# OpenVVC/OpenVVC

Hardware: AMD Instinct MI355X
Metric: decoded frames/sec, full rcn back-end decode step (H2D of the recorded picture + MC incl. BDOF/DMVR/affine-PROF/GPM/CIIP + LMCS + inverse transform + ordered intra pass + deblocking + SAO + ALF/CC-ALF + D2H of refined MVs + wait + per-picture digest + publication to the device DPB), 4K 10-bit RA rec (higher is better)
Workload: dtype u16 samples / int16 coefficients / int32 accumulate

## Files before the change

### include/ovvc_hip.h

```cpp
#ifndef OVVC_HIP_H
#define OVVC_HIP_H

#include <stddef.h>
#include <stdint.h>

#ifdef __cplusplus
extern "C" {
#endif

#define OVHIP_ABI_VERSION 8

#define OVHIP_OK        0
#define OVHIP_ENODEV   (-1)
#define OVHIP_ENOMEM   (-2)
#define OVHIP_EINVAL   (-3)
#define OVHIP_ELAUNCH  (-4)
#define OVHIP_EUNSUP   (-5)
#define OVHIP_EREF     (-6)

enum { OVHIP_DST_VII = 0, OVHIP_DCT_VIII = 1, OVHIP_DCT_II = 2 };

typedef struct ovhip_pic {
    uint16_t *y, *cb, *cr;
    int32_t   w, h;
// ... 358 lines not shown
int   ovhip_rec_cu_inter(ovhip_recorder *rec, const ovhip_pu_desc *pu, const ovhip_affine_desc *aff);
int   ovhip_rec_ciip(ovhip_recorder *rec, int32_t x0, int32_t y0, int32_t log2_w, int32_t log2_h,
                     int32_t mode_abv, int32_t mode_lft);
int   ovhip_ciip_weight(int32_t mode_abv, int32_t mode_lft);
int   ovhip_rec_lmcs_region(ovhip_recorder *rec, int32_t x0, int32_t y0, uint32_t abv_mask, uint32_t lft_mask);
typedef struct ovhip_dbf_edge {
    uint16_t ux, uy;
    uint16_t word;
    uint8_t  comp;
    uint8_t  pad;
} ovhip_dbf_edge;
#define OVHIP_DBF_MAX_OFFSETS 8
typedef struct ovhip_dbf_offsets { int8_t beta[OVHIP_DBF_MAX_OFFSETS], tc[OVHIP_DBF_MAX_OFFSETS]; } ovhip_dbf_offsets;
const ovhip_dbf_edge *ovhip_rec_dbf_edges(const ovhip_recorder *rec, int dir, size_t *n, ovhip_dbf_offsets *offsets);
int64_t ovhip_dbf_compact(const ovhip_dbf_planes *planes, int dir, ovhip_dbf_edge *out, size_t cap);

int   ovhip_rec_dbf_ctu(ovhip_recorder *rec, const ovhip_dbf_ctu *ctu);
typedef struct ovhip_dbf_view {
    const uint64_t *ctb_bound_ver, *ctb_bound_hor, *ctb_bound_ver_c, *ctb_bound_hor_c, *aff_edg_ver, *aff_edg_hor;
    const uint64_t *bs2_ver, *bs2_hor, *bs2c_ver, *bs2c_hor, *bs1_ver, *bs1_hor, *bs1cb_ver, *bs1cb_hor, *bs1cr_ver, *bs1cr_hor, *affine_ver, *affine_hor;
    const uint8_t  *qp_y, *qp_cb, *qp_cr;
    int16_t  beta_offset, tc_offset;
    uint8_t  disable_v, disable_h, log2_ctu_s, last_x, last_y, ctu_lft, ctu_abv, pad;
    uint16_t ctu_w, ctu_h, ctb_x, ctb_y;
} ovhip_dbf_view;
int   ovhip_rec_dbf_row(ovhip_recorder *rec, const ovhip_dbf_view *ctus, size_t n);
int   ovhip_rec_dbf_mv_prepass_view(const ovhip_dbf_view *ctu, uint64_t *bs1_ver, uint64_t *bs1_hor, const ovhip_dbf_mv_ctx *mv);
int   ovhip_rec_dbf_planes(const ovhip_recorder *rec, ovhip_dbf_planes *out);
enum { OVHIP_REC_TB = 0, OVHIP_REC_COEF, OVHIP_REC_MC, OVHIP_REC_MCX, OVHIP_REC_AFF, OVHIP_REC_SIDE, OVHIP_REC_REGION,
       OVHIP_REC_CIIP, OVHIP_REC_EDGE_V, OVHIP_REC_EDGE_H, OVHIP_REC_ITASK };
// ... 368 lines not shown
```

### openvvc_amd/capi.py

```python
from __future__ import annotations

import ctypes as C
import os
from pathlib import Path

import numpy as np

_PKG = Path(__file__).resolve().parent
LIB_PATH = _PKG / os.environ.get("OVVC_HIP_LIB_NAME", "libovvc_hip.so")

OVHIP_ABI_VERSION = 8
OVHIP_OK, OVHIP_ENODEV, OVHIP_ENOMEM, OVHIP_EINVAL, OVHIP_ELAUNCH, OVHIP_EUNSUP, OVHIP_EREF = 0, -1, -2, -3, -4, -5, -6
DST_VII, DCT_VIII, DCT_II = 0, 1, 2
TB_TR, TB_DC, TB_TS, TB_TS_RAW = 0, 1, 2, 3
TB_FLAG_RASTER = 0x80
RES_ADD, RES_SUB, RES_ADD_HALF, RES_SUB_HALF, RES_SCALE = 0, 1, 2, 3, 4
MC_HPEL_FILT, MC_FILT_4x4, MC_NO_LUMA, MC_NO_CHROMA, MC_LMCS, MC_BDOF, MC_DMVR = 1, 2, 4, 8, 16, 32, 64
PU_BDOF, PU_DMVR, PU_GPM = 1, 2, 4
MC_GPM = 128


class Pic(C.Structure):
    _fields_ = [("y", C.c_void_p), ("cb", C.c_void_p), ("cr", C.c_void_p),
                ("w", C.c_int32), ("h", C.c_int32), ("stride_y", C.c_int32), ("stride_c", C.c_int32)]
# ... 161 lines not shown
               [("beta_offset", C.c_int16), ("tc_offset", C.c_int16), ("disable_v", C.c_uint8), ("disable_h", C.c_uint8), ("log2_ctu_s", C.c_uint8),
                ("last_x", C.c_uint8), ("last_y", C.c_uint8), ("ctu_lft", C.c_uint8), ("ctu_abv", C.c_uint8), ("pad", C.c_uint8),
                ("ctu_w", C.c_uint16), ("ctu_h", C.c_uint16), ("ctb_x", C.c_uint16), ("ctb_y", C.c_uint16)]


FE_BEGIN, FE_REF, FE_DMVR_ROWS, FE_DMVR_BEGIN, FE_DMVR_COLLECT, FE_SUBMIT, FE_FAIL = range(1, 8)
FRAME_EVENT_DTYPE = np.dtype([("op", "<u4"), ("frame", "<i4"), ("key", "<u8"), ("tag", "<u8"), ("a", "<i8"), ("b", "<i8"), ("result", "<i8")])
assert FRAME_EVENT_DTYPE.itemsize == 48
FRAME_TRACE_FN = C.CFUNCTYPE(None, C.c_void_p, C.c_void_p)

DBF_PLANE_NAMES = ("luma_v", "luma_h", "cb_v", "cr_v", "cb_h", "cr_h")


class DbfOffsets(C.Structure):
    _fields_ = [("beta", C.c_int8 * 8), ("tc", C.c_int8 * 8)]


class BandCounts(C.Structure):
    _fields_ = [(n, C.c_uint32) for n in ("n_tb", "n_coef", "n_mc", "n_mcx", "n_aff", "n_side", "n_reg", "n_itask", "n_edge_v", "n_edge_h")]


class JobParams(C.Structure):
    _fields_ = [("lmcs", C.c_void_p), ("sao", C.c_void_p), ("alf_ctus", C.c_void_p),
                ("alf_luma_coeff", C.c_void_p), ("alf_luma_clip", C.c_void_p),
                ("alf_chroma_coeff", C.c_void_p), ("alf_chroma_clip", C.c_void_p), ("alf_cc_coeff", C.c_void_p),
                ("log2_ctu_s", C.c_int32), ("stages", C.c_uint32), ("wait_events", C.POINTER(C.c_void_p)), ("n_wait_events", C.c_uint32),
                ("before_launch", C.c_void_p), ("before_launch_user", C.c_void_p), ("tmvp_cells", C.c_uint32), ("wait_on_host", C.c_uint32),
                ("flow_workers", C.c_uint32)]


# ... 210 lines not shown
        "ovhip_d2h": (C.c_int, [vp, vp, vp, C.c_size_t]),
        "ovhip_pic_alloc": (C.c_int, [vp, i32, i32, P(Pic)]),
        "ovhip_pic_free": (C.c_int, [vp, P(Pic)]),
        "ovhip_pic_upload": (C.c_int, [vp, P(Pic), vp, vp, vp, i32, i32]),
        "ovhip_pic_download": (C.c_int, [vp, P(Pic), vp, vp, vp, i32, i32]),
        "ovhip_itx_launch": (C.c_int, [vp, P(Pic), vp, u32, vp, vp]),
        "ovhip_mc_launch": (C.c_int, [vp, P(Pic), P(Pic), u32, vp, u32, vp, P(Pic)]),
        "ovhip_ciip_weight": (C.c_int, [C.c_int32, C.c_int32]),
        "ovhip_mcx_launch": (C.c_int, [vp, P(Pic), P(Pic), u32, vp, u32, vp, vp]),
        "ovhip_mca_launch": (C.c_int, [vp, P(Pic), P(Pic), u32, vp, u32, vp, vp]),
        "ovhip_mcxa_launch": (C.c_int, [vp, P(Pic), P(Pic), u32, vp, u32, vp, vp, u32, vp, vp]),
        "ovhip_rec_create_ex": (vp, [i32, i32, vp]),
        "ovhip_rec_set_dense_dbf_planes": (None, [vp, C.c_int]),
        "ovhip_rec_dbf_edges": (vp, [vp, C.c_int, P(C.c_size_t), P(DbfOffsets)]),
        "ovhip_dbf_launch_edges_ex": (C.c_int, [vp, P(Pic), vp, u32, vp, u32, P(DbfOffsets)]),
        "ovhip_dmvr_search_launch": (C.c_int, [vp, P(Pic), P(Pic), u32, vp, u32, vp]),
        "ovhip_rec_append_raw": (C.c_int, [vp, C.c_int, vp, C.c_size_t]),
        "ovhip_itx_launch_classes_res": (C.c_int, [vp, P(Pic), P(Pic), vp, u32, u32, vp, vp]),
        "ovhip_intra_level_launch": (C.c_int, [vp, P(Pic), P(Pic), vp, u32, vp, vp, vp, i32, u32]),
        "ovhip_intra_level_geom": (u32, [vp, C.c_size_t]),
        "ovhip_intra_sync_words": (C.c_size_t, [i32, i32, i32]),
        "ovhip_intra_flow_words": (C.c_size_t, [i32, i32]),
        "ovhip_intra_flow_items": (C.c_size_t, [vp, C.c_size_t, vp, C.c_size_t]),
        "ovhip_intra_flow_launch": (C.c_int, [vp, P(Pic), P(Pic), vp, u32, vp, u32, vp, vp, vp, i32, vp, u32, vp, i32, i32]),
        "ovhip_intra_ctu_launch": (C.c_int, [vp, P(Pic), P(Pic), vp, vp, u32, vp, vp, vp, i32, vp, u32, vp]),
        "ovhip_rec_itask_levels": (u32, [vp]),
        "ovhip_rec_isp_cu": (C.c_int, [vp, vp, vp]),
        "ovhip_isp_geometry": (None, [i32, i32, i32, P(i32), P(i32), P(i32), P(i32)]),
        "ovhip_job_bind": (C.c_int, [vp, vp]),
        "ovhip_rec_set_ctu_size": (C.c_int, [vp, i32]),
# ... 116 lines not shown
        fn.restype, fn.argtypes = res, args
    if lib.ovhip_abi_version() != OVHIP_ABI_VERSION and not ab_build:
        raise RuntimeError("libovvc_hip.so ABI version mismatch")
    if path is None:
        _lib = lib
    return lib


EXPORTED_SYMBOLS = [
    "ovhip_abi_version", "ovhip_rec_create", "ovhip_rec_destroy", "ovhip_rec_reset", "ovhip_rec_tu",
    "ovhip_rec_pu", "ovhip_rec_cu_inter", "ovhip_rec_dbf_row", "ovhip_rec_dbf_mv_prepass_view", "ovhip_rec_dbf_ctu", "ovhip_rec_dbf_planes", "ovhip_dbf_launch", "ovhip_sao_launch", "ovhip_alf_launch", "ovhip_rec_tb_cmds", "ovhip_rec_coefs", "ovhip_rec_mc_units", "ovhip_rec_mcx_units", "ovhip_mcx_launch", "ovhip_rec_affine_cu", "ovhip_rec_transform_tree", "ovhip_rec_lmcs_region", "ovhip_dbf_compact", "ovhip_rec_dbf_mv_prepass", "ovhip_dbf_launch_edges", "ovhip_rec_ciip", "ovhip_ciip_weight", "ovhip_rec_ciip_units", "ovhip_ciip_launch", "ovhip_rec_lmcs_regions", "ovhip_rec_tb_cmds_split", "ovhip_itx_launch_classes", "ovhip_itx_launch_chroma_lmcs", "ovhip_lmcs_build", "ovhip_lmcs_scale_launch", "ovhip_lmcs_inverse_launch", "ovhip_rec_aff_units", "ovhip_rec_aff_side", "ovhip_mca_launch", "ovhip_mcxa_launch", "ovhip_ctx_create",
    "ovhip_ctx_destroy", "ovhip_ctx_sync", "ovhip_ctx_shares_queue", "ovhip_ctx_new_stream", "ovhip_ctx_fork", "ovhip_ctx_join", "ovhip_last_error", "ovhip_ctx_stream", "ovhip_malloc",
    "ovhip_free", "ovhip_h2d", "ovhip_d2h", "ovhip_pic_alloc", "ovhip_pic_free", "ovhip_pic_upload",
    "ovhip_pic_download", "ovhip_itx_launch", "ovhip_mc_launch",
    "ovhip_rec_create_ex", "ovhip_rec_set_dense_dbf_planes", "ovhip_rec_dbf_edges", "ovhip_dbf_launch_edges_ex",
    "ovhip_dmvr_search_launch", "ovhip_rec_append_raw", "ovhip_rec_set_dbf_offsets", "ovhip_rec_tu_intra", "ovhip_rec_itasks", "ovhip_rec_itasks_sorted", "ovhip_itx_launch_classes_res", "ovhip_intra_level_launch", "ovhip_intra_level_geom", "ovhip_intra_sync_words", "ovhip_intra_ctu_launch", "ovhip_intra_flow_words", "ovhip_intra_flow_items", "ovhip_intra_flow_launch",
    "ovhip_rec_itask_levels", "ovhip_rec_isp_cu", "ovhip_isp_geometry", "ovhip_rec_itasks_by_ctu", "ovhip_rec_set_ctu_size", "ovhip_job_bind", "ovhip_job_create", "ovhip_job_destroy", "ovhip_job_recorder", "ovhip_job_begin",
    "ovhip_frame_band", "ovhip_frame_band_upto", "ovhip_frame_dmvr_rows_begin_upto", "ovhip_job_dmvr_rows_begin_upto", "ovhip_frame_set_band_mode", "ovhip_frame_band_stats", "ovhip_dpb_post_rows", "ovhip_dpb_rows_tag",
    "ovhip_job_band", "ovhip_job_band_active", "ovhip_job_band_busy", "ovhip_job_band_reserve", "ovhip_job_reserve_for_picture", "ovhip_rec_reserve_for_picture", "ovhip_job_band_progress", "ovhip_rec_counts", "ovhip_sao_launch_rows", "ovhip_alf_launch_rows",
    "ovhip_job_flush", "ovhip_job_wait", "ovhip_job_refined_mvs", "ovhip_job_dmvr_rows", "ovhip_job_dmvr_rows_begin", "ovhip_job_dmvr_rows_collect", "ovhip_job_last_stats", "ovhip_job_time_stage", "ovhip_job_stage_time",
    "ovhip_output_bytes", "ovhip_output_rows", "ovhip_output_pack_launch", "ovhip_output_row_md5_launch", "ovhip_output_bands", "ovhip_output_tree_md5_launch", "ovhip_pic_output", "ovhip_pic_digest",
    "ovhip_md5_init", "ovhip_md5_update", "ovhip_md5_final", "ovhip_tmvp_cells_launch", "ovhip_job_tmvp_cells", "ovhip_intra_flow_untag_launch", "ovhip_lmcs_inverse_untag_launch", "ovhip_lmcs_scale_prepare_launch",
    "ovhip_host_alloc", "ovhip_host_free", "ovhip_d2d", "ovhip_job_test_abort_next_flow",
    "ovhip_dpb_create", "ovhip_dpb_create_ex", "ovhip_dpb_destroy", "ovhip_dpb_n_devices", "ovhip_dpb_device", "ovhip_dpb_begin", "ovhip_dpb_want",
    "ovhip_dpb_publish", "ovhip_dpb_acquire", "ovhip_dpb_wait_copy", "ovhip_dpb_poll_tag", "ovhip_frame_refs_ready", "ovhip_dpb_set_unknown_key_timeout", "ovhip_dpb_unpin", "ovhip_dpb_release", "ovhip_dpb_lookup", "ovhip_dpb_shutdown",
    "ovhip_dpb_get_stats", "ovhip_dpb_begin_tag", "ovhip_dpb_want_tag", "ovhip_dpb_acquire_tag", "ovhip_frame_begin_tag", "ovhip_frame_ref_tag", "ovhip_frame_set_trace",
    "ovhip_rccl_unique_id", "ovhip_rccl_create", "ovhip_rccl_destroy", "ovhip_rccl_xfer", "ovhip_rccl_last_error", "ovhip_rccl_stats", "ovhip_rccl_self_exchange",
    "ovhip_frame_create", "ovhip_frame_destroy", "ovhip_frame_ctx", "ovhip_frame_job", "ovhip_frame_recorder", "ovhip_frame_begin", "ovhip_frame_ref",
    "ovhip_frame_ref_at", "ovhip_frame_dmvr_rows", "ovhip_frame_dmvr_rows_begin", "ovhip_frame_dmvr_rows_collect", "ovhip_frame_submit", "ovhip_frame_fail", "ovhip_frame_last_error",
    "ovhip_calllog_create", "ovhip_calllog_destroy", "ovhip_calllog_reset", "ovhip_calllog_data", "ovhip_rec_set_calllog", "ovhip_calllog_replay",
# ... 217 lines not shown
```

### openvvc_amd/csrc/kernels_dbf.hip

```cpp
#include "ovvc_common.hip.h"
#define OVT_ATTR __device__
#include "vvc_dbf_tables.h"

#ifndef OV_WPE_DBF
#define OV_WPE_DBF 0
#endif
#if OV_WPE_DBF > 0
#define OV_OCC_DBF __attribute__((amdgpu_waves_per_eu(OV_WPE_DBF)))
#else
#define OV_OCC_DBF
#endif

namespace {

struct Lim { int tc, beta; };

__device__ __forceinline__ Lim dbf_limits(int qp, int bs, int tc_off, int beta_off)
{
    Lim l;
    l.tc = ovt_dbf_tc[ov_clip3(qp + 2 * (bs - 1) + tc_off, 0, 66)];
    l.beta = (int)ovt_dbf_beta[ov_clip3(qp + beta_off, 0, 64)] << 2;
    return l;
}

// ... 308 lines not shown
        const int cw = DIR ? w4 : (w4 + 1) >> 1, chh = DIR ? (h4 + 1) >> 1 : h4;
        const uint16_t *plane = DIR ? (comp == 1 ? pl.cb_h : pl.cr_h) : (comp == 1 ? pl.cb_v : pl.cr_v);
        for (int tid = blockIdx.x * 256 + threadIdx.x; tid < cw * chh; tid += nthreads) {
            const int cx = tid % cw, cy = tid / cw;
            const int v = plane[tid];
            if (!(v & OVHIP_DBF_C_ON)) continue;
            const int ux = DIR ? cx : cx * 2, uy = DIR ? cy * 2 : cy;
            if ((DIR ? uy : ux) == 0) continue;
            const Lim lim = dbf_limits(v >> 8, 1 + !!(v & OVHIP_DBF_C_BS2), pl.tc_offset, pl.beta_offset);
            uint16_t *p = (comp == 1 ? pic.cb : pic.cr) + (uy * 2) * pic.stride_c + ux * 2;
            chroma_segment(p, DIR ? pic.stride_c : 1, DIR ? 1 : pic.stride_c, lim, v & OVHIP_DBF_C_LARGE, v & OVHIP_DBF_C_CTB_B);
        }
    }
}

template <int DIR>
__global__ __launch_bounds__(256) OV_OCC_DBF void k_dbf_list(ovhip_pic pic, const ovhip_dbf_edge *__restrict__ edges, uint32_t n,
                                                  uint64_t tc_pack, uint64_t beta_pack)
{
    const uint32_t tid = ov_xcd_slot(blockIdx.x, gridDim.x) * 256 + threadIdx.x;
    const uint32_t ei = tid >> 2;
    const int l = tid & 3;
    if (ei >= n) return;
    const ovhip_dbf_edge e = edges[ei];
    const int v = e.word;
    const int osh = (e.pad & 7) * 8;
    const int tc_offset = (int8_t)(tc_pack >> osh), beta_offset = (int8_t)(beta_pack >> osh);
    if (e.comp == 0) {
        const Lim lim = dbf_limits(v >> 8, v & 3, tc_offset, beta_offset);
        if (!(lim.tc || lim.beta)) return;
        uint16_t *p = pic.y + (e.uy * 4) * pic.stride_y + e.ux * 4 + l * (DIR ? 1 : pic.stride_y);
        luma_quad<DIR>(p, DIR ? pic.stride_y : 1, lim, (v >> 2) & 7, (v >> 5) & 7);
    } else {
        const Lim lim = dbf_limits(v >> 8, 1 + !!(v & OVHIP_DBF_C_BS2), tc_offset, beta_offset);
        uint16_t *p = (e.comp == 1 ? pic.cb : pic.cr) + (e.uy * 2) * pic.stride_c + e.ux * 2 + (l & 1) * (DIR ? 1 : pic.stride_c);
        chroma_quad<DIR>(p, DIR ? pic.stride_c : 1, lim, v & OVHIP_DBF_C_LARGE, v & OVHIP_DBF_C_CTB_B, l < 2);
    }
}

}

extern "C" int ovhip_dbf_launch_edges_ex(ovhip_ctx *ctx, const ovhip_pic *pic, const ovhip_dbf_edge *d_edges_v, uint32_t n_v,
                                         const ovhip_dbf_edge *d_edges_h, uint32_t n_h, const ovhip_dbf_offsets *offsets)
{
    if (!ctx || !pic || !offsets) return OVHIP_EINVAL;
    OV_DEVICE(ctx);
    if ((n_v && !d_edges_v) || (n_h && !d_edges_h))
        return ov_fail(ctx, OVHIP_EINVAL, "ovhip_dbf_launch_edges: null edge list", hipSuccess);
    uint64_t tc_pack, beta_pack;
    memcpy(&tc_pack, offsets->tc, 8); memcpy(&beta_pack, offsets->beta, 8);
    if (n_v) {
        hipLaunchKernelGGL(k_dbf_list<0>, dim3((n_v + 63) / 64), dim3(256), 0, ctx->stream, *pic, d_edges_v, n_v, tc_pack, beta_pack);
        OV_LAUNCH_CHECK(ctx, "k_dbf_list<v>");
    }
    if (n_h) {
        hipLaunchKernelGGL(k_dbf_list<1>, dim3((n_h + 63) / 64), dim3(256), 0, ctx->stream, *pic, d_edges_h, n_h, tc_pack, beta_pack);
        OV_LAUNCH_CHECK(ctx, "k_dbf_list<h>");
    }
    return OVHIP_OK;
}

extern "C" int ovhip_dbf_launch_edges(ovhip_ctx *ctx, const ovhip_pic *pic, const ovhip_dbf_edge *d_edges_v, uint32_t n_v,
                                      const ovhip_dbf_edge *d_edges_h, uint32_t n_h, int32_t beta_offset, int32_t tc_offset)
{
    if (beta_offset < -128 || beta_offset > 127 || tc_offset < -128 || tc_offset > 127) return OVHIP_EINVAL;
    ovhip_dbf_offsets o;
    for (int i = 0; i < OVHIP_DBF_MAX_OFFSETS; ++i) { o.beta[i] = (int8_t)beta_offset; o.tc[i] = (int8_t)tc_offset; }
    return ovhip_dbf_launch_edges_ex(ctx, pic, d_edges_v, n_v, d_edges_h, n_h, &o);
}

extern "C" int ovhip_dbf_launch(ovhip_ctx *ctx, const ovhip_pic *pic, const ovhip_dbf_planes *pl)
{
    if (!ctx || !pic || !pl) return OVHIP_EINVAL;
    OV_DEVICE(ctx);
// ... 14 lines not shown
```

### openvvc_amd/csrc/ovvc_picture.hip

```cpp
#include "ovvc_common.hip.h"
#include <stdlib.h>

extern "C" int ovhip_dmvr_search_launch(ovhip_ctx *ctx, const ovhip_pic *geom, const ovhip_pic *refs, uint32_t n_refs,
                                        const ovhip_mc_unit *d_units, uint32_t n_units, int32_t *d_mv_out);

struct BandState;
namespace {

struct DevBuf { void *p; size_t cap; };

enum { B_TB, B_COEF, B_MC, B_MCX, B_MV, B_AFF, B_SIDE, B_REG, B_SCALE, B_EV, B_EH, B_PARAM, B_CLASS, B_CIIP, B_ITASK, B_ICTU, B_IITEM, B_TMVP, B_COUNT };

struct ParamLayout { size_t sao, alf_ctus, lcoef, lclip, ccoef, cclip, cc, fwd, bwd, total; };

}

struct ovhip_job {
    ovhip_ctx *ctx;
    ovhip_ctx *home;
    int32_t w, h;
    ovhip_recorder *rec;
    DevBuf dev[B_COUNT];
    ovhip_pic tmp;
    ovhip_pic res;
// ... 5 lines not shown
    int32_t *mv_host; size_t mv_cap;
    struct { int valid, has_intra; ovhip_pic dst, refs[16], intra; uint32_t n_refs; ovhip_job_params pr; } again;
    uint32_t n_retries;
    int flow_launched;
    int test_abort, test_abort_seen;
    ovhip_tmvp_cell *tmvp_host; size_t tmvp_cap, n_tmvp;
    size_t n_mv;
    size_t dmvr_first;
    size_t rows_end; int rows_pending;
    hipEvent_t ev_rows;
    hipEvent_t ev_h2d, ev_done;
    hipStream_t up;
    int flow_on_device;
    int flushed;
    const void *packed_prev[24];
    int resident;
    ovhip_job_stats st;
    struct BandState *bs;
    int t_stage;
    hipEvent_t t_ev[32][2]; uint8_t t_pending[32]; int t_next;
    double t_sum_ms; uint64_t t_count;
};

static void band_free(ovhip_job *j);
static int  band_reset(ovhip_job *j);
static int  band_active(const ovhip_job *j);
static int  band_wait_done(ovhip_job *j);

enum { FLOW_DEVS = 64, FLOW_DECAY = 512 };
static int g_flow_shift[FLOW_DEVS], g_flow_clean[FLOW_DEVS];
// ... 88 lines not shown
    return OVHIP_OK;
}

int pinned_reserve(ovhip_job *j, void **p, size_t *cap, size_t bytes)
{
    if (bytes <= *cap) return OVHIP_OK;
    size_t nc = *cap ? *cap : 4096;
    while (nc < bytes) nc *= 2;
    void *q = pinned_alloc(nullptr, nc);
    if (!q) return ov_fail(j->ctx, OVHIP_ENOMEM, "hipHostMalloc", hipSuccess);
    if (*p) { memcpy(q, *p, *cap); pinned_free(nullptr, *p); }
    *p = q; *cap = nc;
    return OVHIP_OK;
}

extern "C" const ovhip_tb_cmd *ovhip_rec_tb_cmds_split_tiny_(ovhip_recorder *r, size_t counts[4], size_t tiny[4][4], size_t *n);
extern "C" int ovhip_itx_launch_ex_(ovhip_ctx *ctx, const ovhip_pic *dst, const ovhip_pic *res, const ovhip_tb_cmd *d_cmds, uint32_t n_large,
                                    uint32_t n_small, const uint32_t tiny3[4], const int16_t *d_coefs, const int16_t *d_lmcs_scales, const uint16_t *d_bwd_lut);

#define CHK(x) do { int r__ = (x); if (r__ != OVHIP_OK) return r__; } while (0)

#ifndef OVHIP_PACK_LIMIT
#define OVHIP_PACK_LIMIT (1 << 20)
#endif

double host_now_us()
{
    timespec t;
    clock_gettime(CLOCK_MONOTONIC, &t);
    return 1e6 * (double)t.tv_sec + 1e-3 * (double)t.tv_nsec;
// ... 401 lines not shown
    const int sao_on = pr->sao && (stages & OVHIP_STAGE_SAO), alf_on = pr->alf_ctus && (stages & OVHIP_STAGE_ALF);
    if (alf_on && (!pr->alf_luma_coeff || !pr->alf_luma_clip || !pr->alf_chroma_coeff || !pr->alf_chroma_clip || !pr->alf_cc_coeff))
        return ov_fail(ctx, OVHIP_EINVAL, "ovhip_job_flush: ALF tables missing", hipSuccess);
    ParamLayout L;
    size_t o = 0;
    auto put = [&o](size_t bytes) { size_t at = o; o += (bytes + 255) & ~(size_t)255; return at; };
    L.sao = put(sao_on ? n_ctu * sizeof(ovhip_sao_ctu) : 0);
    L.alf_ctus = put(alf_on ? n_ctu * sizeof(ovhip_alf_ctu) : 0);
    L.lcoef = put(alf_on ? 24 * OVHIP_ALF_LUMA_SET_SIZE * 2 : 0);
    L.lclip = put(alf_on ? 24 * OVHIP_ALF_LUMA_SET_SIZE * 2 : 0);
    L.ccoef = put(alf_on ? 8 * 7 * 2 : 0);
    L.cclip = put(alf_on ? 8 * 7 * 2 : 0);
    L.cc = put(alf_on ? 2 * 4 * 8 * 2 : 0);
    L.fwd = put(pr->lmcs ? 2048 : 0);
    L.bwd = put(pr->lmcs ? 2048 : 0);
#ifdef OVHIP_TUNING
    static const size_t PACK_LIMIT = getenv("OVHIP_X_PACK_LIMIT") ? (size_t)atol(getenv("OVHIP_X_PACK_LIMIT")) : (size_t)OVHIP_PACK_LIMIT;
#else
    const size_t PACK_LIMIT = OVHIP_PACK_LIMIT;
#endif
    struct Small { const void *host; size_t bytes; int buf; size_t at; } small[] = {
        { mc, n_mc * sizeof(*mc), B_MC, 0 }, { tb, n_tb * sizeof(*tb), B_TB, 0 }, { coef, n_coef * sizeof(*coef), B_COEF, 0 },
        { it, n_it * sizeof(*it), B_ITASK, 0 }, { ictu, n_ictu * sizeof(*ictu), B_ICTU, 0 },
        { j->items_host, by_flow ? n_items * sizeof(uint32_t) : 0, B_IITEM, 0 },
        { mcx, n_mcx * sizeof(*mcx), B_MCX, 0 }, { ciip, n_ciip * sizeof(*ciip), B_CIIP, 0 }, { aff, n_aff * sizeof(*aff), B_AFF, 0 },
        { side, n_side * sizeof(*side), B_SIDE, 0 }, { reg, n_reg * sizeof(*reg), B_REG, 0 },
        { ev, (stages & OVHIP_STAGE_DBF) ? n_ev * sizeof(*ev) : 0, B_EV, 0 }, { eh, (stages & OVHIP_STAGE_DBF) ? n_eh * sizeof(*eh) : 0, B_EH, 0 },
    };
    static_assert(B_COUNT <= 24, "packed_prev");
    const void *packed[24] = { nullptr };
    for (auto &sm : small) if (sm.bytes && sm.bytes <= PACK_LIMIT && !j->resident) sm.at = put(sm.bytes) + 1;
    L.total = o;
    if (L.total) {
        CHK(pinned_reserve(j, (void **)&j->param_host, &j->param_cap, L.total));
        char *ph = j->param_host;
        for (auto &sm : small) if (sm.at) memcpy(ph + sm.at - 1, sm.host, sm.bytes);
        if (sao_on) memcpy(ph + L.sao, pr->sao, n_ctu * sizeof(ovhip_sao_ctu));
        if (alf_on) {
            memcpy(ph + L.alf_ctus, pr->alf_ctus, n_ctu * sizeof(ovhip_alf_ctu));
            memcpy(ph + L.lcoef, pr->alf_luma_coeff, 24 * OVHIP_ALF_LUMA_SET_SIZE * 2);
            memcpy(ph + L.lclip, pr->alf_luma_clip, 24 * OVHIP_ALF_LUMA_SET_SIZE * 2);
            memcpy(ph + L.ccoef, pr->alf_chroma_coeff, 8 * 7 * 2);
            memcpy(ph + L.cclip, pr->alf_chroma_clip, 8 * 7 * 2);
            memcpy(ph + L.cc, pr->alf_cc_coeff, 2 * 4 * 8 * 2);
        }
        if (pr->lmcs) { memcpy(ph + L.fwd, pr->lmcs->fwd_lut, 2048); memcpy(ph + L.bwd, pr->lmcs->bwd_lut, 2048); }
    }

    const double t_flush1 = host_now_us();
    j->up = (j->resident || no_upload) ? nullptr : upload_stream_for(j);
    if (j->up) {
        hipError_t e0 = hipSuccess;
        if (j->flushed) e0 = hipStreamWaitEvent(j->up, j->ev_done, 0);
        if (e0 == hipSuccess && j->rows_pending) e0 = hipStreamWaitEvent(j->up, j->ev_rows, 0);
        if (e0 != hipSuccess) { j->up = nullptr; return ov_fail(ctx, OVHIP_ENODEV, "ovhip_job_flush: upload stream", e0); }
    }
    {
    StageTimer t_(j, OVHIP_TIME_H2D);
    CHK(h2d(j, B_PARAM, j->param_host, L.total));
    if (n_mcx) {
        CHK(dev_reserve(j, B_MV, n_mcx * 16));
        CHK(pinned_reserve(j, (void **)&j->mv_host, &j->mv_cap, n_mcx * 16));
    }
    if (n_reg) CHK(dev_reserve(j, B_SCALE, n_reg * 2));
    for (auto &sm : small) {
        if (j->resident) continue;
        if (sm.at) packed[sm.buf] = (const char *)j->dev[B_PARAM].p + sm.at - 1;
        else CHK(h2d(j, sm.buf, sm.host, sm.bytes));
    }
    }
    if (no_upload) memcpy(packed, j->packed_prev, sizeof(packed)); else { memcpy(j->packed_prev, packed, sizeof(packed)); j->flow_on_device = by_flow && n_items; }
    auto DEV = [&](int k) -> const void * { return packed[k] ? packed[k] : j->dev[k].p; };
    if (j->up) {
        hipStream_t up = j->up; j->up = nullptr;
        OV_HIP(ctx, hipEventRecord(j->ev_h2d, up));
        OV_HIP(ctx, hipStreamWaitEvent(ctx->stream, j->ev_h2d, 0));
    } else OV_HIP(ctx, hipEventRecord(j->ev_h2d, ctx->stream));
    const double t_flush2 = host_now_us();
    for (uint32_t i = 0; i < pr->n_wait_events; ++i)
        if (pr->wait_events && pr->wait_events[i]) {
            if (pr->wait_on_host) OV_HIP(ctx, hipEventSynchronize((hipEvent_t)pr->wait_events[i]));
            else OV_HIP(ctx, hipStreamWaitEvent(ctx->stream, (hipEvent_t)pr->wait_events[i], 0));
        }
    if (pr->before_launch && pr->before_launch(pr->before_launch_user))
        return ov_fail(ctx, OVHIP_EINVAL, "ovhip_job_flush: before_launch callback failed", hipSuccess);
#ifdef OVHIP_TUNING
    static const int X_H2D_HOSTWAIT = getenv("OVHIP_X_H2D_HOSTWAIT") ? atoi(getenv("OVHIP_X_H2D_HOSTWAIT")) : 0;
    static const int X_MV_D2H = getenv("OVHIP_X_MV_D2H") ? atoi(getenv("OVHIP_X_MV_D2H")) : 3;
    if (X_H2D_HOSTWAIT && !j->resident) OV_HIP(ctx, hipEventSynchronize(j->ev_h2d));
#else
    const int X_MV_D2H = 3;
#endif
// ... 139 lines not shown
        }
        for (uint32_t l = 0; by_level && !by_flow && l < n_lv; ++l) {
            const uint32_t a = lv_start[l], b = lv_start[l + 1];
            if (b > a) {
                CHK(ovhip_intra_level_launch(ctx, dst, &j->res, d_it + a, b - a, (const ovhip_lmcs_region *)DEV(B_REG), pr->lmcs,
                                             (int16_t *)j->dev[B_SCALE].p, log2_ctu, ovhip_intra_level_geom(it + a, b - a)));
                j->st.n_launches++;
            }
        }
        const bool inverse = pr->lmcs && (stages & OVHIP_STAGE_ITX);
        if (inverse) { CHK(ovhip_lmcs_inverse_untag_launch(ctx, dst, d_bwd, d_it, by_flow && n_items ? (uint32_t)n_it : 0u)); j->st.n_launches++; }
        else if (by_flow && n_items) { CHK(ovhip_intra_flow_untag_launch(ctx, dst, d_it, (uint32_t)n_it, 1)); j->st.n_launches++; }
    }
    if (stages & OVHIP_STAGE_DBF) {
        StageTimer t_(j, OVHIP_TIME_DBF);
        CHK(ovhip_dbf_launch_edges_ex(ctx, dst, (const ovhip_dbf_edge *)DEV(B_EV), (uint32_t)n_ev,
                                      (const ovhip_dbf_edge *)DEV(B_EH), (uint32_t)n_eh, &offs));
        j->st.n_launches += (n_ev != 0) + (n_eh != 0);
    }
    if (sao_on) {
        StageTimer t_(j, OVHIP_TIME_SAO);
        CHK(ovhip_sao_launch(ctx, &j->tmp, dst, (const ovhip_sao_ctu *)(dp + L.sao), log2_ctu));
        j->st.n_launches++;
    }
    if (alf_on) {
        CHK(dev_reserve(j, B_CLASS, (size_t)((j->w + 3) / 4) * ((j->h + 3) / 4)));
        ovhip_alf_pic ap;
        ap.ctus = (const ovhip_alf_ctu *)(dp + L.alf_ctus);
        ap.luma_coeff = (const int16_t *)(dp + L.lcoef); ap.luma_clip = (const int16_t *)(dp + L.lclip);
        ap.chroma_coeff = (const int16_t *)(dp + L.ccoef); ap.chroma_clip = (const int16_t *)(dp + L.cclip);
        ap.cc_coeff = (const int16_t *)(dp + L.cc);
        ap.class_scratch = (uint8_t *)j->dev[B_CLASS].p;
// ... 553 lines not shown
```

### openvvc_amd/csrc/ovvc_record_dbf.c

```c
#include <stdlib.h>
#include <string.h>
#include "ovvc_hip.h"
#include "ovvc_record_priv.h"

static int
dbf_alloc(ovhip_recorder *r)
{
    const int w4 = (r->pic_w + 3) >> 2, h4 = (r->pic_h + 3) >> 2;
    const int w4c = (w4 + 1) >> 1, h4c = (h4 + 1) >> 1;
    r->dbf_w4 = w4; r->dbf_h4 = h4;
    if (r->dbf_luma_v || !r->dense_planes) return 0;
    r->dbf_luma_v = (uint16_t *)calloc((size_t)w4 * h4, 2);
    r->dbf_luma_h = (uint16_t *)calloc((size_t)w4 * h4, 2);
    r->dbf_cb_v = (uint16_t *)calloc((size_t)w4c * h4, 2);
    r->dbf_cr_v = (uint16_t *)calloc((size_t)w4c * h4, 2);
    r->dbf_cb_h = (uint16_t *)calloc((size_t)w4 * h4c, 2);
    r->dbf_cr_h = (uint16_t *)calloc((size_t)w4 * h4c, 2);
    if (!r->dbf_luma_v || !r->dbf_luma_h || !r->dbf_cb_v || !r->dbf_cr_v || !r->dbf_cb_h || !r->dbf_cr_h) return -1;
    return 0;
}

void
ovhip_rec_dbf_reset_(ovhip_recorder *r)
{
// ... 274 lines not shown
            }
        }
    }
    return OVHIP_OK;
}

const ovhip_dbf_edge *
ovhip_rec_dbf_edges(const ovhip_recorder *r, int dir, size_t *n, ovhip_dbf_offsets *offsets)
{
    if (!r || !n || (dir != 0 && dir != 1)) return NULL;
    *n = dir ? r->n_edge_h : r->n_edge_v;
    if (offsets) *offsets = r->dbf_off;
    return dir ? r->edge_h : r->edge_v;
}

int64_t
ovhip_dbf_compact(const ovhip_dbf_planes *pl, int dir, ovhip_dbf_edge *out, size_t cap)
{
    if (!pl || (dir != 0 && dir != 1) || pl->w4 <= 0 || pl->h4 <= 0) return OVHIP_EINVAL;
    const int w4 = pl->w4, h4 = pl->h4;
    size_t n = 0;
    const uint16_t *luma = dir ? pl->luma_h : pl->luma_v;
    if (!luma) return OVHIP_EINVAL;
    for (int uy = 0; uy < h4; ++uy)
        for (int ux = 0; ux < w4; ++ux) {
            const uint16_t v = luma[uy * w4 + ux];
            if (!(v & 3) || (dir ? uy : ux) == 0) continue;
            if (out && n < cap) { ovhip_dbf_edge e = { (uint16_t)ux, (uint16_t)uy, v, 0, 0 }; out[n] = e; }
            ++n;
        }
// ... 130 lines not shown
```

Measured before the change: 3575.

## Pack deblocking edge lists into compact 32-bit wire format for upload

Adds a band-chunked 32-bit encoding of deblocking edges, with one row band per 64-entry chunk and packed ux/uy/comp/word fields. The encoded lists go into the pinned parameter buffer, so they ride the single H2D copy instead of separate 8-byte-per-edge uploads. The DBF kernel gets a WIRE template variant that decodes the words on device. The host pays an extra encode pass per picture and some padding slots. It falls back to the raw edge lists when fields don't fit, such as nonzero offset index or wide coordinates.

```diff
diff --git a/include/ovvc_hip.h b/include/ovvc_hip.h
--- a/include/ovvc_hip.h
+++ b/include/ovvc_hip.h
@@ -396,6 +396,11 @@
 typedef struct ovhip_dbf_offsets { int8_t beta[OVHIP_DBF_MAX_OFFSETS], tc[OVHIP_DBF_MAX_OFFSETS]; } ovhip_dbf_offsets;
 const ovhip_dbf_edge *ovhip_rec_dbf_edges(const ovhip_recorder *rec, int dir, size_t *n, ovhip_dbf_offsets *offsets);
 int64_t ovhip_dbf_compact(const ovhip_dbf_planes *planes, int dir, ovhip_dbf_edge *out, size_t cap);
+#define OVHIP_DBF_WIRE_CHUNK 64
+typedef struct ovhip_dbf_wire { uint32_t n_slots, words_off; } ovhip_dbf_wire;
+size_t  ovhip_dbf_wire_bound(size_t n, int32_t pic_h);
+int64_t ovhip_dbf_wire_encode(const ovhip_dbf_edge *edges, size_t n, int32_t pic_h, void *out, size_t cap, ovhip_dbf_wire *w);
+int64_t ovhip_dbf_wire_decode(const void *in, const ovhip_dbf_wire *w, ovhip_dbf_edge *out, size_t cap);
 
 int   ovhip_rec_dbf_ctu(ovhip_recorder *rec, const ovhip_dbf_ctu *ctu);
 typedef struct ovhip_dbf_view {
diff --git a/openvvc_amd/capi.py b/openvvc_amd/capi.py
--- a/openvvc_amd/capi.py
+++ b/openvvc_amd/capi.py
@@ -199,6 +199,10 @@
 
 class DbfOffsets(C.Structure):
     _fields_ = [("beta", C.c_int8 * 8), ("tc", C.c_int8 * 8)]
+
+
+class DbfWire(C.Structure):
+    _fields_ = [("n_slots", C.c_uint32), ("words_off", C.c_uint32)]
 
 
 class BandCounts(C.Structure):
@@ -439,6 +443,9 @@
         "ovhip_rec_set_dense_dbf_planes": (None, [vp, C.c_int]),
         "ovhip_rec_dbf_edges": (vp, [vp, C.c_int, P(C.c_size_t), P(DbfOffsets)]),
         "ovhip_dbf_launch_edges_ex": (C.c_int, [vp, P(Pic), vp, u32, vp, u32, P(DbfOffsets)]),
+        "ovhip_dbf_wire_bound": (C.c_size_t, [C.c_size_t, i32]),
+        "ovhip_dbf_wire_encode": (C.c_int64, [vp, C.c_size_t, i32, vp, C.c_size_t, P(DbfWire)]),
+        "ovhip_dbf_wire_decode": (C.c_int64, [vp, P(DbfWire), vp, C.c_size_t]),
         "ovhip_dmvr_search_launch": (C.c_int, [vp, P(Pic), P(Pic), u32, vp, u32, vp]),
         "ovhip_rec_append_raw": (C.c_int, [vp, C.c_int, vp, C.c_size_t]),
         "ovhip_itx_launch_classes_res": (C.c_int, [vp, P(Pic), P(Pic), vp, u32, u32, vp, vp]),
@@ -585,6 +592,7 @@
     "ovhip_free", "ovhip_h2d", "ovhip_d2h", "ovhip_pic_alloc", "ovhip_pic_free", "ovhip_pic_upload",
     "ovhip_pic_download", "ovhip_itx_launch", "ovhip_mc_launch",
     "ovhip_rec_create_ex", "ovhip_rec_set_dense_dbf_planes", "ovhip_rec_dbf_edges", "ovhip_dbf_launch_edges_ex",
+    "ovhip_dbf_wire_bound", "ovhip_dbf_wire_encode", "ovhip_dbf_wire_decode",
     "ovhip_dmvr_search_launch", "ovhip_rec_append_raw", "ovhip_rec_set_dbf_offsets", "ovhip_rec_tu_intra", "ovhip_rec_itasks", "ovhip_rec_itasks_sorted", "ovhip_itx_launch_classes_res", "ovhip_intra_level_launch", "ovhip_intra_level_geom", "ovhip_intra_sync_words", "ovhip_intra_ctu_launch", "ovhip_intra_flow_words", "ovhip_intra_flow_items", "ovhip_intra_flow_launch",
     "ovhip_rec_itask_levels", "ovhip_rec_isp_cu", "ovhip_isp_geometry", "ovhip_rec_itasks_by_ctu", "ovhip_rec_set_ctu_size", "ovhip_job_bind", "ovhip_job_create", "ovhip_job_destroy", "ovhip_job_recorder", "ovhip_job_begin",
     "ovhip_frame_band", "ovhip_frame_band_upto", "ovhip_frame_dmvr_rows_begin_upto", "ovhip_job_dmvr_rows_begin_upto", "ovhip_frame_set_band_mode", "ovhip_frame_band_stats", "ovhip_dpb_post_rows", "ovhip_dpb_rows_tag",
diff --git a/openvvc_amd/csrc/kernels_dbf.hip b/openvvc_amd/csrc/kernels_dbf.hip
--- a/openvvc_amd/csrc/kernels_dbf.hip
+++ b/openvvc_amd/csrc/kernels_dbf.hip
@@ -346,50 +346,82 @@
     }
 }
 
-template <int DIR>
-__global__ __launch_bounds__(256) OV_OCC_DBF void k_dbf_list(ovhip_pic pic, const ovhip_dbf_edge *__restrict__ edges, uint32_t n,
-                                                  uint64_t tc_pack, uint64_t beta_pack)
+template <int DIR, bool WIRE>
+__global__ __launch_bounds__(256) OV_OCC_DBF void k_dbf_list(ovhip_pic pic, const void *__restrict__ list, uint32_t n,
+                                                  const uint16_t *__restrict__ bands, uint64_t tc_pack, uint64_t beta_pack)
 {
     const uint32_t tid = ov_xcd_slot(blockIdx.x, gridDim.x) * 256 + threadIdx.x;
     const uint32_t ei = tid >> 2;
     const int l = tid & 3;
     if (ei >= n) return;
-    const ovhip_dbf_edge e = edges[ei];
-    const int v = e.word;
-    const int osh = (e.pad & 7) * 8;
+    int ux, uy, comp, v, osh;
+    if (WIRE) {
+        const uint32_t w = static_cast<const uint32_t *>(list)[ei];
+        comp = (w >> 15) & 3;
+        if (comp == 3) return;
+        const int p = w & 0x7fff;
+        ux = w >> 22; uy = bands[ei / OVHIP_DBF_WIRE_CHUNK] * 32 + ((w >> 17) & 31);
+        v = comp ? (p & 15) | ((p >> 4) << 8) : ((p & ~1) << 1) | (1 + (p & 1));
+        osh = 0;
+    } else {
+        const ovhip_dbf_edge e = static_cast<const ovhip_dbf_edge *>(list)[ei];
+        ux = e.ux; uy = e.uy; comp = e.comp; v = e.word;
+        osh = (e.pad & 7) * 8;
+    }
     const int tc_offset = (int8_t)(tc_pack >> osh), beta_offset = (int8_t)(beta_pack >> osh);
-    if (e.comp == 0) {
+    if (comp == 0) {
         const Lim lim = dbf_limits(v >> 8, v & 3, tc_offset, beta_offset);
         if (!(lim.tc || lim.beta)) return;
-        uint16_t *p = pic.y + (e.uy * 4) * pic.stride_y + e.ux * 4 + l * (DIR ? 1 : pic.stride_y);
+        uint16_t *p = pic.y + (uy * 4) * pic.stride_y + ux * 4 + l * (DIR ? 1 : pic.stride_y);
         luma_quad<DIR>(p, DIR ? pic.stride_y : 1, lim, (v >> 2) & 7, (v >> 5) & 7);
     } else {
         const Lim lim = dbf_limits(v >> 8, 1 + !!(v & OVHIP_DBF_C_BS2), tc_offset, beta_offset);
-        uint16_t *p = (e.comp == 1 ? pic.cb : pic.cr) + (e.uy * 2) * pic.stride_c + e.ux * 2 + (l & 1) * (DIR ? 1 : pic.stride_c);
+        uint16_t *p = (comp == 1 ? pic.cb : pic.cr) + (uy * 2) * pic.stride_c + ux * 2 + (l & 1) * (DIR ? 1 : pic.stride_c);
         chroma_quad<DIR>(p, DIR ? pic.stride_c : 1, lim, v & OVHIP_DBF_C_LARGE, v & OVHIP_DBF_C_CTB_B, l < 2);
     }
 }
 
+template <int DIR>
+int dbf_list_launch(ovhip_ctx *ctx, const ovhip_pic *pic, const void *d_list, uint32_t n, const ovhip_dbf_wire *wire,
+                    uint64_t tc_pack, uint64_t beta_pack)
+{
+    if (wire) {
+        const uint16_t *bands = static_cast<const uint16_t *>(d_list);
+        const void *words = static_cast<const char *>(d_list) + wire->words_off;
+        hipLaunchKernelGGL((k_dbf_list<DIR, true>), dim3((wire->n_slots + 63) / 64), dim3(256), 0, ctx->stream, *pic, words, wire->n_slots,
+                           bands, tc_pack, beta_pack);
+    } else {
+        hipLaunchKernelGGL((k_dbf_list<DIR, false>), dim3((n + 63) / 64), dim3(256), 0, ctx->stream, *pic, d_list, n,
+                           (const uint16_t *)nullptr, tc_pack, beta_pack);
+    }
+    OV_LAUNCH_CHECK(ctx, DIR ? "k_dbf_list<h>" : "k_dbf_list<v>");
+    return OVHIP_OK;
+}
+
+}
+
+extern "C" int ovhip_dbf_launch_lists_(ovhip_ctx *ctx, const ovhip_pic *pic, const void *d_v, uint32_t n_v, const ovhip_dbf_wire *wire_v,
+                                       const void *d_h, uint32_t n_h, const ovhip_dbf_wire *wire_h, const ovhip_dbf_offsets *offsets)
+{
+    if (!ctx || !pic || !offsets) return OVHIP_EINVAL;
+    OV_DEVICE(ctx);
+    if (wire_v && !wire_v->n_slots) wire_v = nullptr, n_v = 0;
+    if (wire_h && !wire_h->n_slots) wire_h = nullptr, n_h = 0;
+    if ((n_v && !d_v) || (n_h && !d_h) || (wire_v && !d_v) || (wire_h && !d_h))
+        return ov_fail(ctx, OVHIP_EINVAL, "ovhip_dbf_launch_edges: null edge list", hipSuccess);
+    if ((wire_v && (wire_v->words_off & 3)) || (wire_h && (wire_h->words_off & 3)))
+        return ov_fail(ctx, OVHIP_EINVAL, "ovhip_dbf_launch_edges: misaligned wire form", hipSuccess);
+    uint64_t tc_pack, beta_pack;
+    memcpy(&tc_pack, offsets->tc, 8); memcpy(&beta_pack, offsets->beta, 8);
+    if (n_v || wire_v) { const int r = dbf_list_launch<0>(ctx, pic, d_v, n_v, wire_v, tc_pack, beta_pack); if (r) return r; }
+    if (n_h || wire_h) { const int r = dbf_list_launch<1>(ctx, pic, d_h, n_h, wire_h, tc_pack, beta_pack); if (r) return r; }
+    return OVHIP_OK;
 }
 
 extern "C" int ovhip_dbf_launch_edges_ex(ovhip_ctx *ctx, const ovhip_pic *pic, const ovhip_dbf_edge *d_edges_v, uint32_t n_v,
                                          const ovhip_dbf_edge *d_edges_h, uint32_t n_h, const ovhip_dbf_offsets *offsets)
 {
-    if (!ctx || !pic || !offsets) return OVHIP_EINVAL;
-    OV_DEVICE(ctx);
-    if ((n_v && !d_edges_v) || (n_h && !d_edges_h))
-        return ov_fail(ctx, OVHIP_EINVAL, "ovhip_dbf_launch_edges: null edge list", hipSuccess);
-    uint64_t tc_pack, beta_pack;
-    memcpy(&tc_pack, offsets->tc, 8); memcpy(&beta_pack, offsets->beta, 8);
-    if (n_v) {
-        hipLaunchKernelGGL(k_dbf_list<0>, dim3((n_v + 63) / 64), dim3(256), 0, ctx->stream, *pic, d_edges_v, n_v, tc_pack, beta_pack);
-        OV_LAUNCH_CHECK(ctx, "k_dbf_list<v>");
-    }
-    if (n_h) {
-        hipLaunchKernelGGL(k_dbf_list<1>, dim3((n_h + 63) / 64), dim3(256), 0, ctx->stream, *pic, d_edges_h, n_h, tc_pack, beta_pack);
-        OV_LAUNCH_CHECK(ctx, "k_dbf_list<h>");
-    }
-    return OVHIP_OK;
+    return ovhip_dbf_launch_lists_(ctx, pic, d_edges_v, n_v, nullptr, d_edges_h, n_h, nullptr, offsets);
 }
 
 extern "C" int ovhip_dbf_launch_edges(ovhip_ctx *ctx, const ovhip_pic *pic, const ovhip_dbf_edge *d_edges_v, uint32_t n_v,
diff --git a/openvvc_amd/csrc/ovvc_picture.hip b/openvvc_amd/csrc/ovvc_picture.hip
--- a/openvvc_amd/csrc/ovvc_picture.hip
+++ b/openvvc_amd/csrc/ovvc_picture.hip
@@ -43,6 +43,7 @@
     int flow_on_device;
     int flushed;
     const void *packed_prev[24];
+    ovhip_dbf_wire wire_prev[2];
     int resident;
     ovhip_job_stats st;
     struct BandState *bs;
@@ -161,6 +162,18 @@
     return OVHIP_OK;
 }
 
+static int wire_enabled()
+{
+    static int on = -1;
+    if (__atomic_load_n(&on, __ATOMIC_RELAXED) < 0) {
+        const char *e = getenv("OVVC_HIP_WIRE");
+        __atomic_store_n(&on, e ? atoi(e) != 0 : 1, __ATOMIC_RELAXED);
+    }
+    return __atomic_load_n(&on, __ATOMIC_RELAXED);
+}
+
+extern "C" int ovhip_dbf_launch_lists_(ovhip_ctx *ctx, const ovhip_pic *pic, const void *d_v, uint32_t n_v, const ovhip_dbf_wire *wire_v,
+                                       const void *d_h, uint32_t n_h, const ovhip_dbf_wire *wire_h, const ovhip_dbf_offsets *offsets);
 extern "C" const ovhip_tb_cmd *ovhip_rec_tb_cmds_split_tiny_(ovhip_recorder *r, size_t counts[4], size_t tiny[4][4], size_t *n);
 extern "C" int ovhip_itx_launch_ex_(ovhip_ctx *ctx, const ovhip_pic *dst, const ovhip_pic *res, const ovhip_tb_cmd *d_cmds, uint32_t n_large,
                                     uint32_t n_small, const uint32_t tiny3[4], const int16_t *d_coefs, const int16_t *d_lmcs_scales, const uint16_t *d_bwd_lut);
@@ -592,6 +605,19 @@
     L.cc = put(alf_on ? 2 * 4 * 8 * 2 : 0);
     L.fwd = put(pr->lmcs ? 2048 : 0);
     L.bwd = put(pr->lmcs ? 2048 : 0);
+    ovhip_dbf_wire wire[2] = { { 0, 0 }, { 0, 0 } };
+    size_t wire_at[2] = { 0, 0 };
+    if (!j->resident && (stages & OVHIP_STAGE_DBF) && wire_enabled() && (n_ev || n_eh)) {
+        const size_t bv = ovhip_dbf_wire_bound(n_ev, j->h), bh = ovhip_dbf_wire_bound(n_eh, j->h);
+        CHK(pinned_reserve(j, (void **)&j->param_host, &j->param_cap, o + bv + 256 + bh));
+        for (int d = 0; d < 2; ++d) {
+            const size_t n_d = d ? n_eh : n_ev;
+            if (!n_d) continue;
+            const int64_t r = ovhip_dbf_wire_encode(d ? eh : ev, n_d, j->h, j->param_host + o, d ? bh : bv, &wire[d]);
+            if (r > 0) wire_at[d] = put((size_t)r) + 1;
+            else wire[d].n_slots = 0;
+        }
+    }
 #ifdef OVHIP_TUNING
     static const size_t PACK_LIMIT = getenv("OVHIP_X_PACK_LIMIT") ? (size_t)atol(getenv("OVHIP_X_PACK_LIMIT")) : (size_t)OVHIP_PACK_LIMIT;
 #else
@@ -603,7 +629,8 @@
         { j->items_host, by_flow ? n_items * sizeof(uint32_t) : 0, B_IITEM, 0 },
         { mcx, n_mcx * sizeof(*mcx), B_MCX, 0 }, { ciip, n_ciip * sizeof(*ciip), B_CIIP, 0 }, { aff, n_aff * sizeof(*aff), B_AFF, 0 },
         { side, n_side * sizeof(*side), B_SIDE, 0 }, { reg, n_reg * sizeof(*reg), B_REG, 0 },
-        { ev, (stages & OVHIP_STAGE_DBF) ? n_ev * sizeof(*ev) : 0, B_EV, 0 }, { eh, (stages & OVHIP_STAGE_DBF) ? n_eh * sizeof(*eh) : 0, B_EH, 0 },
+        { ev, (stages & OVHIP_STAGE_DBF) && !wire_at[0] ? n_ev * sizeof(*ev) : 0, B_EV, 0 },
+        { eh, (stages & OVHIP_STAGE_DBF) && !wire_at[1] ? n_eh * sizeof(*eh) : 0, B_EH, 0 },
     };
     static_assert(B_COUNT <= 24, "packed_prev");
     const void *packed[24] = { nullptr };
@@ -633,27 +660,31 @@
         if (e0 == hipSuccess && j->rows_pending) e0 = hipStreamWaitEvent(j->up, j->ev_rows, 0);
         if (e0 != hipSuccess) { j->up = nullptr; return ov_fail(ctx, OVHIP_ENODEV, "ovhip_job_flush: upload stream", e0); }
     }
-    {
-    StageTimer t_(j, OVHIP_TIME_H2D);
-    CHK(h2d(j, B_PARAM, j->param_host, L.total));
-    if (n_mcx) {
-        CHK(dev_reserve(j, B_MV, n_mcx * 16));
-        CHK(pinned_reserve(j, (void **)&j->mv_host, &j->mv_cap, n_mcx * 16));
-    }
-    if (n_reg) CHK(dev_reserve(j, B_SCALE, n_reg * 2));
-    for (auto &sm : small) {
-        if (j->resident) continue;
-        if (sm.at) packed[sm.buf] = (const char *)j->dev[B_PARAM].p + sm.at - 1;
-        else CHK(h2d(j, sm.buf, sm.host, sm.bytes));
-    }
-    }
-    if (no_upload) memcpy(packed, j->packed_prev, sizeof(packed)); else { memcpy(j->packed_prev, packed, sizeof(packed)); j->flow_on_device = by_flow && n_items; }
-    auto DEV = [&](int k) -> const void * { return packed[k] ? packed[k] : j->dev[k].p; };
+    int up_rc = OVHIP_OK;
+    do {
+        StageTimer t_(j, OVHIP_TIME_H2D);
+        if ((up_rc = h2d(j, B_PARAM, j->param_host, L.total))) break;
+        if (n_mcx) {
+            if ((up_rc = dev_reserve(j, B_MV, n_mcx * 16))) break;
+            if ((up_rc = pinned_reserve(j, (void **)&j->mv_host, &j->mv_cap, n_mcx * 16))) break;
+        }
+        if (n_reg && (up_rc = dev_reserve(j, B_SCALE, n_reg * 2))) break;
+        for (auto &sm : small) {
+            if (j->resident) continue;
+            if (sm.at) packed[sm.buf] = (const char *)j->dev[B_PARAM].p + sm.at - 1;
+            else if ((up_rc = h2d(j, sm.buf, sm.host, sm.bytes))) break;
+        }
+        for (int d = 0; d < 2; ++d) if (wire_at[d]) packed[d ? B_EH : B_EV] = (const char *)j->dev[B_PARAM].p + wire_at[d] - 1;
+    } while (0);
     if (j->up) {
         hipStream_t up = j->up; j->up = nullptr;
         OV_HIP(ctx, hipEventRecord(j->ev_h2d, up));
         OV_HIP(ctx, hipStreamWaitEvent(ctx->stream, j->ev_h2d, 0));
     } else OV_HIP(ctx, hipEventRecord(j->ev_h2d, ctx->stream));
+    if (up_rc) return up_rc;
+    if (no_upload) { memcpy(packed, j->packed_prev, sizeof(packed)); memcpy(wire, j->wire_prev, sizeof(wire)); }
+    else { memcpy(j->packed_prev, packed, sizeof(packed)); memcpy(j->wire_prev, wire, sizeof(wire)); j->flow_on_device = by_flow && n_items; }
+    auto DEV = [&](int k) -> const void * { return packed[k] ? packed[k] : j->dev[k].p; };
     const double t_flush2 = host_now_us();
     for (uint32_t i = 0; i < pr->n_wait_events; ++i)
         if (pr->wait_events && pr->wait_events[i]) {
@@ -823,8 +854,8 @@
     }
     if (stages & OVHIP_STAGE_DBF) {
         StageTimer t_(j, OVHIP_TIME_DBF);
-        CHK(ovhip_dbf_launch_edges_ex(ctx, dst, (const ovhip_dbf_edge *)DEV(B_EV), (uint32_t)n_ev,
-                                      (const ovhip_dbf_edge *)DEV(B_EH), (uint32_t)n_eh, &offs));
+        CHK(ovhip_dbf_launch_lists_(ctx, dst, DEV(B_EV), (uint32_t)n_ev, wire[0].n_slots ? &wire[0] : nullptr,
+                                    DEV(B_EH), (uint32_t)n_eh, wire[1].n_slots ? &wire[1] : nullptr, &offs));
         j->st.n_launches += (n_ev != 0) + (n_eh != 0);
     }
     if (sao_on) {
diff --git a/openvvc_amd/csrc/ovvc_record_dbf.c b/openvvc_amd/csrc/ovvc_record_dbf.c
--- a/openvvc_amd/csrc/ovvc_record_dbf.c
+++ b/openvvc_amd/csrc/ovvc_record_dbf.c
@@ -312,6 +312,86 @@
     return dir ? r->edge_h : r->edge_v;
 }
 
+#define WIRE_NULL (3u << 15)
+
+static size_t
+wire_slots_cap(size_t n, int32_t pic_h)
+{
+    const size_t bands = ((size_t)(pic_h > 0 ? pic_h : 0) + 127) >> 7;
+    return (n + OVHIP_DBF_WIRE_CHUNK * (2 * bands + 2) + OVHIP_DBF_WIRE_CHUNK - 1) & ~(size_t)(OVHIP_DBF_WIRE_CHUNK - 1);
+}
+
+static size_t wire_words_off(size_t slots_cap) { return ((slots_cap / OVHIP_DBF_WIRE_CHUNK) * 2 + 15) & ~(size_t)15; }
+
+size_t
+ovhip_dbf_wire_bound(size_t n, int32_t pic_h)
+{
+    const size_t s = wire_slots_cap(n, pic_h);
+    return wire_words_off(s) + 4 * s;
+}
+
+__attribute__((target_clones("avx2", "default"))) int64_t
+ovhip_dbf_wire_encode(const ovhip_dbf_edge *e, size_t n, int32_t pic_h, void *out, size_t cap, ovhip_dbf_wire *w)
+{
+    if ((n && !e) || !out || !w) return OVHIP_EINVAL;
+    const size_t slots_cap = wire_slots_cap(n, pic_h), words_off = wire_words_off(slots_cap);
+    if (cap < words_off + 4 * slots_cap) return OVHIP_EINVAL;
+    uint16_t *band = (uint16_t *)out;
+    uint32_t *word = (uint32_t *)((char *)out + words_off);
+    const uint64_t *in = (const uint64_t *)e;
+    uint64_t bad = 0;
+    size_t i = 0, s = 0;
+    while (i < n) {
+        if (s >= slots_cap) return OVHIP_EUNSUP;
+        const uint64_t cur = (in[i] >> 21) & 0x7ff;
+        band[s / OVHIP_DBF_WIRE_CHUNK] = (uint16_t)cur;
+        const size_t k = n - i < OVHIP_DBF_WIRE_CHUNK ? n - i : OVHIP_DBF_WIRE_CHUNK;
+        const uint32_t *in32 = (const uint32_t *)(in + i);
+        uint32_t *dst = word + s, bad32 = 0, other = 0;
+        for (size_t j = 0; j < k; ++j) {
+            const uint32_t a = in32[2 * j], b = in32[2 * j + 1];
+            const uint32_t ux = a & 0xffff, uy = a >> 16, v = b & 0xffff, comp = (b >> 16) & 0xff;
+            const uint32_t chroma = 0u - (comp != 0);
+            const uint32_t p = (((v & 15) | ((v >> 8) << 4)) & chroma) | ((v >> 1) & ~chroma);
+            bad32 |= (v & 0xf0 & chroma) | (((((v & 3) + 1) & 2) ^ 2) & ~chroma) | (ux >> 10) | (comp > 2) | (b >> 24);
+            other |= (uy >> 5) ^ (uint32_t)cur;
+            dst[j] = ux << 22 | (uy & 31u) << 17 | comp << 15 | p;
+        }
+        bad |= bad32;
+        if (!other) { i += k; s += k; continue; }
+        size_t j = 0;
+        while (((in[i + j] >> 21) & 0x7ff) == cur) ++j;
+        i += j; s += j;
+        while (s & (OVHIP_DBF_WIRE_CHUNK - 1)) word[s++] = WIRE_NULL;
+    }
+    if (bad) return OVHIP_EUNSUP;
+    w->n_slots = (uint32_t)s; w->words_off = (uint32_t)words_off;
+    return (int64_t)(words_off + 4 * s);
+}
+
+int64_t
+ovhip_dbf_wire_decode(const void *in, const ovhip_dbf_wire *w, ovhip_dbf_edge *out, size_t cap)
+{
+    if (!in || !w || (w->words_off & 3)) return OVHIP_EINVAL;
+    const uint16_t *band = (const uint16_t *)in;
+    const uint32_t *word = (const uint32_t *)((const char *)in + w->words_off);
+    size_t n = 0;
+    for (size_t s = 0; s < w->n_slots; ++s) {
+        const uint32_t x = word[s], comp = (x >> 15) & 3, p = x & 0x7fff;
+        if (comp == 3) continue;
+        if (out && n < cap) {
+            ovhip_dbf_edge d;
+            d.ux = (uint16_t)(x >> 22);
+            d.uy = (uint16_t)(band[s / OVHIP_DBF_WIRE_CHUNK] * 32 + ((x >> 17) & 31));
+            d.word = (uint16_t)(comp ? (p & 15) | ((p >> 4) << 8) : ((p & ~1u) << 1) | (1 + (p & 1)));
+            d.comp = (uint8_t)comp; d.pad = 0;
+            out[n] = d;
+        }
+        ++n;
+    }
+    return (int64_t)n;
+}
+
 int64_t
 ovhip_dbf_compact(const ovhip_dbf_planes *pl, int dir, ovhip_dbf_edge *out, size_t cap)
 {
```

New measurement: 3640 (median of 6 runs). No clear change (+1.8%).
